# apchenstu/mvsnerf

Hardware: AMD Instinct MI355X
Metric: rendered rays/sec (1024-ray batch, 128 samples) (higher is better)
Workload: dtype f32; 1 GPU; config 2: 3 source views 512x640, 128 depth planes, pad 24 (volume 128x176x208x8), 1024 rays x 128 samples per step, MLP arithmetic fp32, render-only (volume pre-built); weights=mvsnerf-v0 checkpoint, volume=mvsnet-encode, parallelism=ray-sharded x1, no data-path collective

## Files before the change

mvsnerf_amd/csrc/mlp.hip:

```cpp
#include "common.h"
#include "mlp_layout.h"
#include "lds_dma.h"
#include "mlp_fp32_dev.h"
#include "knobs.h"
#include "sample_dev.h"
#include "composite_wave.h"
#include "march.h"

using namespace mlp;
typedef float f32x2 __attribute__((ext_vector_type(2)));

struct PackArgs {
    const float* w[11];
    const float* b[11];
    int F;
    float add;
};

__device__ inline void pack_segment(float* __restrict__ dst, const float* __restrict__ W, int ld, int col_off,
                                    int kmap, int steps, int nb, int F, int tid, int nthreads)
{
    const int total = steps * nb * 64;
    for (int i = tid; i < total; i += nthreads) {
        const int j = i & 3;
        const int lane = (i >> 2) & 63;
        const int rest = i >> 8;
        const int b = rest % nb, t = (rest / nb) * 4 + j;
        const int col = kmap_col(kmap, t, lane >> 5, F);
        const int row = b * 32 + (lane & 31);
        dst[i] = col < 0 ? 0.0f : W[(size_t)row * ld + col_off + col];
    }
}

template <bool FOLD>
__global__ __launch_bounds__(256) void mlp_pack_kernel(PackArgs a, float* __restrict__ packed)
{
    const Layout L = layout(a.F);
    const int tid = blockIdx.x * blockDim.x + threadIdx.x, nt = gridDim.x * blockDim.x;
    pack_segment(packed + L.biasw, a.w[6], a.F, 0, K_FEAT, L.fsteps, 4, a.F, tid, nt);
    pack_segment(packed + L.l0, a.w[0], PE_DIM, 0, K_PE, PE_STEPS, 4, a.F, tid, nt);
    pack_segment(packed + L.l1, a.w[1], WIDTH, 0, K_ACT, ACT_STEPS, 4, a.F, tid, nt);
    pack_segment(packed + L.l2, a.w[2], WIDTH, 0, K_ACT, ACT_STEPS, 4, a.F, tid, nt);
    pack_segment(packed + L.l3, a.w[3], WIDTH, 0, K_ACT, ACT_STEPS, 4, a.F, tid, nt);
    pack_segment(packed + L.l4, a.w[4], WIDTH, 0, K_ACT, ACT_STEPS, 4, a.F, tid, nt);
    pack_segment(packed + L.l5a, a.w[5], WIDTH + PE_DIM, 0, K_PE, PE_STEPS, 4, a.F, tid, nt);
    pack_segment(packed + L.l5b, a.w[5], WIDTH + PE_DIM, PE_DIM, K_ACT, ACT_STEPS, 4, a.F, tid, nt);
    pack_segment(packed + L.feat, a.w[7], WIDTH, 0, K_ACT, ACT_STEPS, 4, a.F, tid, nt);
    pack_segment(packed + L.views, a.w[9], WIDTH + 3, 0, K_VIEWS, VIEW_STEPS, 2, a.F, tid, nt);
    float* v = packed + L.vec;
    for (int i = tid; i < V_TOTAL; i += nt) {
        float x = 0.0f;
        if (i < V_VIEWS) {
            const int which = i >> 7, h = (i >> 6) & 1, q = i & 63;
            const float* src = which == 0 ? a.b[6] : which <= 6 ? a.b[which - 1] : a.b[7];
            x = src[act_n(q, h)];
        } else if (i < V_WA) {
            const int k = i - V_VIEWS;
            x = a.b[9][act_n(k & 31, k >> 5)];
        } else if (i < V_BA) {
            const int k = i - V_WA;
            x = a.w[8][act_n(k & 63, k >> 6)];
        } else if (i < V_WR) {
            x = (i == V_BA) ? a.b[8][0] : (FOLD && i == V_FOLD) ? 1.0f : (i == V_ADD) ? a.add : 0.0f;
        } else if (i < V_BR) {
            const int k = i - V_WR, c = k >> 6, h = (k >> 5) & 1, q = k & 31;
            x = a.w[10][c * 64 + act_n(q, h)];
        } else {
            const int c = i - V_BR;
            x = c < 3 ? a.b[10][c] : 0.0f;
        }
        v[i] = x;
    }
    if constexpr (FOLD) {
        const float* Wv = a.w[9];
        const float* Wf = a.w[7];
        float* fw = packed + fold_views_off(a.F);
        float* fb = packed + fold_bias_off(a.F);
        constexpr int total = (int)seg_floats(VIEW_STEPS, 2);
        for (int i = tid; i < total + 64; i += nt) {
            if (i < total) {
                const int lane = (i >> 2) & 63, rest = i >> 8;
                const int t = (rest >> 1) * 4 + (i & 3);
                const int col = kmap_col(K_VIEWS, t, lane >> 5, a.F);
                const float* wrow = Wv + (size_t)((rest & 1) * 32 + (lane & 31)) * (WIDTH + 3);
                float x = 0.0f;
                if (col >= WIDTH) {
                    x = wrow[col];
                } else if (col >= 0) {
                    double acc = 0.0;
                    for (int j = 0; j < WIDTH; ++j) acc = acc + (double)wrow[j] * (double)Wf[j * WIDTH + col];
                    x = (float)acc;
                }
                fw[i] = x;
            } else {
                const int k = i - total, n = act_n(k & 31, k >> 5);
                double acc = (double)a.b[9][n];
                for (int j = 0; j < WIDTH; ++j) acc = acc + (double)Wv[(size_t)n * (WIDTH + 3) + j] * (double)a.b[7][j];
                fb[k] = (float)acc;
            }
        }
    }
}

static size_t off16(int F) { return (layout(F).total + 3) & ~(size_t)3; }

extern "C" size_t mvsnerf_mlp_packed_floats(int F)
{
    if (F < 2 || F > MAX_F || (F & 1)) return 0;
    return off16(F);
}

extern "C" size_t mvsnerf_mlp_packed_fold_floats(int F)
{
    if (F < 2 || F > MAX_F || (F & 1)) return 0;
    return fold_total(F);
}

template <bool FOLD>
static int mlp_pack_impl(const float* const w[11], const float* const b[11], int F, float* packed, void* stream, float add = 0.0f)
{
    if (!w || !b || !packed) return MVSNERF_EINVAL;
    if (F < 2 || F > MAX_F || (F & 1)) return MVSNERF_EUNSUPPORTED;
    if (!mvs_aligned16(packed)) return MVSNERF_EALIGN;
    PackArgs a;
    for (int i = 0; i < 11; ++i) {
        if (!w[i] || !b[i]) return MVSNERF_EINVAL;
        a.w[i] = w[i]; a.b[i] = b[i];
    }
    a.F = F;
    a.add = add;
    mlp_pack_kernel<FOLD><<<64, 256, 0, (hipStream_t)stream>>>(a, packed);
    MVS_LAUNCH_CHECK();
    return MVSNERF_OK;
}

extern "C" int mvsnerf_mlp_pack(const float* const w[11], const float* const b[11], int F, float* packed, void* stream)
{
    return mlp_pack_impl<false>(w, b, F, packed, stream);
}

extern "C" int mvsnerf_mlp_pack_fold(const float* const w[11], const float* const b[11], int F, float* packed, void* stream)
{
    return mlp_pack_impl<true>(w, b, F, packed, stream);
}

extern "C" int mvsnerf_mlp_pack_fold_variant(const float* const w[11], const float* const b[11], int F, int variant, float* packed, void* stream)
{
    if (variant != 0 && variant != 1) return MVSNERF_EINVAL;
    return mlp_pack_impl<true>(w, b, F, packed, stream, variant ? 1.0f : 0.0f);
}

constexpr int WBUF_FLOATS = 16384;
constexpr int LDS_FLOATS = WBUF_FLOATS + V_TOTAL;

__device__ __forceinline__ void stage_weights(float* __restrict__ wbuf, const float* __restrict__ src, int n_floats, int tid)
{
    const f32x4* s = reinterpret_cast<const f32x4*>(src);
    f32x4* d = reinterpret_cast<f32x4*>(wbuf);
    const int n4 = n_floats >> 2;
#pragma unroll 4
    for (int i = tid; i < n4; i += 256) d[i] = s[i];
}

constexpr int SLAB_FLOATS = 8704;
constexpr int PIPE_LDS_FLOATS = 2 * SLAB_FLOATS + V_TOTAL;

struct RaymarchTileArgs {
    const float* vol; int D, H, W;
    const float* img; int V, IH, IW;
    const float* w2c; const float* Kmat;
    const float* pts; const float* rays_dir;
    float* feat; float* dirs_out;
    const float* z; int64_t N; int rays_per_tile;
    CompositeOut o;
};

__device__ __forceinline__ void tile_lookups(const unsigned tile, const RaymarchTileArgs& a, const float* __restrict__ ndc, int64_t P, int F,
                                             float* __restrict__ stage)
{
#pragma clang fp contract(off)
    const int tid = threadIdx.x, q = tid & 3;
    int r[2];
    bool live[2];
    unsigned p[2];
    ZfastTaps zt[2];
    ColorTap ct[2][2];
    f32x3 tap[2][2][4];
    f32x3 nn[2], pp[2];
#pragma unroll
    for (int ps = 0; ps < 2; ++ps) {
        r[ps] = ps * 64 + (tid >> 2);
        const int64_t p_raw = (int64_t)tile * 128 + r[ps];
        live[ps] = p_raw < P;
        p[ps] = (unsigned)(live[ps] ? p_raw : P - 1);
        nn[ps] = f32x3{ndc[p[ps] * 3 + 0], ndc[p[ps] * 3 + 1], ndc[p[ps] * 3 + 2]};
        pp[ps] = *reinterpret_cast<const f32x3*>(a.pts + p[ps] * 3);
    }
    const bool two = a.V > 4;
    const int vk[2] = {q < a.V ? q : a.V - 1, q + 4 < a.V ? q + 4 : a.V - 1};
    float Mv[2][12], Kv[2][9];
#pragma unroll
    for (int k = 0; k < 2; ++k)
        if (k == 0 || two) {
#pragma unroll
            for (int i = 0; i < 12; ++i) Mv[k][i] = a.w2c[vk[k] * 16 + i];
#pragma unroll
            for (int i = 0; i < 9; ++i) Kv[k][i] = a.Kmat[vk[k] * 9 + i];
        }
#pragma unroll
    for (int ps = 0; ps < 2; ++ps) zt[ps] = zfast_taps<true>(a.vol, a.D, a.H, a.W, nn[ps][0], nn[ps][1], nn[ps][2], q);
#pragma unroll
    for (int ps = 0; ps < 2; ++ps)
#pragma unroll
        for (int k = 0; k < 2; ++k)
            if (k == 0 || two) {
                ct[ps][k] = color_project(pp[ps][0], pp[ps][1], pp[ps][2], Mv[k], Kv[k], a.IW, a.IH);
                color_taps_nhwc4<true, f32x3>(a.img, vk[k], a.IH, a.IW, ct[ps][k], tap[ps][k]);
            }
#pragma unroll
    for (int ps = 0; ps < 2; ++ps) {
        float* srow = stage + r[ps] * F;
#pragma unroll
        for (int k = 0; k < 2; ++k)
            if ((k == 0 || two) && q + 4 * k < a.V) *reinterpret_cast<f32x4*>(srow + 8 + 16 * k + 4 * q) = color_row(ct[ps][k], tap[ps][k]);
        const f32x4 acc = zfast_fold_y0_lane(zt[ps]);
        if (q < 2) *reinterpret_cast<f32x4*>(srow + q * 4) = acc;
    }
}

__device__ __forceinline__ void tile_rows_out(const unsigned tile, float* __restrict__ feat, const float* __restrict__ stage, int64_t P, int F)
{
    const int64_t row0 = (int64_t)tile * 128;
    const int n4 = (int)(P - row0 < 128 ? P - row0 : 128) * (F / 4);
    f32x4* dst = reinterpret_cast<f32x4*>(feat + row0 * F);
    const f32x4* src = reinterpret_cast<const f32x4*>(stage);
    for (int i = threadIdx.x; i < n4; i += 256) dst[i] = src[i];
}

template <bool ALPHA_ONLY, bool SAVE, bool FUSED = false, int NR = 0>
__device__ __forceinline__ void mlp_fwd_pipe_tile(
    const unsigned tile, const float* __restrict__ packed, int F, const float* __restrict__ ndc, int ndc_stride,
    const float* __restrict__ feat, int feat_stride, const float* __restrict__ dirs, int dirs_stride,
    int64_t P, int S, float* __restrict__ raw, float* __restrict__ saved, long long* __restrict__ census, const RaymarchTileArgs* fa = nullptr)
{
    extern __shared__ __attribute__((aligned(16))) float lds[];
    long long t_start = 0, c_start = 0;
    if (census) { t_start = wall_clock64(); c_start = __builtin_amdgcn_s_memtime(); }
    int stamp_i = 4;
    auto stamp = [&]() { if (census && threadIdx.x == 0 && stamp_i < 16) census[tile * 16 + stamp_i] = wall_clock64(); ++stamp_i; };
    float* buf0 = lds;
    float* buf1 = lds + SLAB_FLOATS;
    float* vec = lds + 2 * SLAB_FLOATS;
    constexpr int G = 1;
    const Layout L = layout(F);
    const int tid = threadIdx.x, lane = tid & 63;
    const int wave = __builtin_amdgcn_readfirstlane(tid >> 6);
    const int half = lane >> 5;
    const int64_t p_raw = ((int64_t)tile * 4 + wave) * 32 + (lane & 31);
    const bool live = p_raw < P;
    const int64_t p = live ? p_raw : P - 1;
    float* sv = nullptr;
    if (SAVE) sv = saved + ((int64_t)tile * 4 + wave) * (SLOTS_SAVED * 64) + lane;
    auto save = [&](int slot, float v) { if (SAVE) sv[slot * 64] = v; };
    constexpr int HALF = (int)(ACT_STEPS / 2) * 4 * 64;

    constexpr int VEC_PER_THREAD = (V_TOTAL + 255) / 256;
    float vec_pre[VEC_PER_THREAD];
    if constexpr (FUSED) {
#pragma unroll
        for (int k = 0; k < VEC_PER_THREAD; ++k) vec_pre[k] = tid + 256 * k < V_TOTAL ? packed[L.vec + tid + 256 * k] : 0.0f;
    }
    slab_dma(buf0, packed + L.biasw, (int)seg_floats(L.fsteps, 4), wave, lane);
    const bool l0_first = !FUSED || seg_floats(L.fsteps, 4) + 128 * (size_t)F <= SLAB_FLOATS;
    float* stage = l0_first ? buf0 + seg_floats(L.fsteps, 4) : buf1;
    if (l0_first) slab_dma_c<(int)seg_floats(PE_STEPS, 4)>(buf1, packed + L.l0, wave, lane);
    if constexpr (FUSED) {
        tile_lookups(tile, *fa, ndc, P, F, stage);
#pragma unroll
        for (int k = 0; k < VEC_PER_THREAD; ++k)
            if (tid + 256 * k < V_TOTAL) vec[tid + 256 * k] = vec_pre[k];
    } else {
        for (int i = tid; i < V_TOTAL; i += 256) vec[i] = packed[L.vec + i];
    }
    const float px = ndc[p * ndc_stride + 0], py = ndc[p * ndc_stride + 1], pz = ndc[p * ndc_stride + 2];
    float fv[MAX_F / 2];
    if constexpr (FUSED) {
        slab_sync();
        const float* fp = stage + (wave * 32 + (lane & 31)) * F + half * (F / 2);
#pragma unroll
        for (int i = 0; i < MAX_F / 2; ++i) fv[i] = i < F / 2 ? fp[i] : 0.0f;
        tile_rows_out(tile, fa->feat, stage, P, F);
        if (!l0_first) {
            __syncthreads();
            slab_dma_c<(int)seg_floats(PE_STEPS, 4)>(buf1, packed + L.l0, wave, lane);
        }
    } else {
        const float* fp = feat + p * feat_stride + half * (F / 2);
#pragma unroll
        for (int i = 0; i < MAX_F / 2; ++i) fv[i] = i < F / 2 ? fp[i] : 0.0f;
    }
    float bias[64], h[64], pe_e[PE_STEPS];
    auto pe = [&](int g, int t) { return pe_e[t]; };
    auto hlo = [&](int g, int t) { return h[t]; };
    auto hhi = [&](int g, int t) { return h[32 + t]; };

    if constexpr (!FUSED) slab_sync();
    constexpr bool MAY_FOLD = !ALPHA_ONLY && !SAVE;
    bool fold = false;
    if constexpr (MAY_FOLD) {
        fold = __builtin_amdgcn_readfirstlane(__float_as_int(vec[V_FOLD])) != 0;
        if (fold && wave == 0) lds_dma_dword(packed + fold_bias_off(F), lds_byte_addr(vec + V_VIEWS), lane * 4);
    }
    const bool add = __builtin_amdgcn_readfirstlane(__float_as_int(vec[V_ADD])) != 0;
    stamp();
    {
        f32x16 acc[G][4];
        init_acc<4, G>(acc, vec + V_BIASG + half * 64);
        auto fb = [&](int g, int t) { return fv[t]; };
        switch (L.fsteps) {
            case 4:  gemm_stage<1, 4, G>(buf0, acc, lane, fb); break;
            case 8:  gemm_stage<2, 4, G>(buf0, acc, lane, fb); break;
            case 12: gemm_stage<3, 4, G>(buf0, acc, lane, fb); break;
            case 16: gemm_stage<4, 4, G>(buf0, acc, lane, fb); break;
            default: gemm_stage<5, 4, G>(buf0, acc, lane, fb); break;
        }
#pragma unroll
        for (int q = 0; q < 64; ++q) { bias[q] = acc[0][q >> 4][q & 15]; save(S_BM + q, bias[q]); }
        if (SAVE) {
#pragma unroll
            for (int t = 0; t < 16; ++t) save(S_FV + t, fv[t]);
            if (F > 32) {
#pragma unroll
                for (int t = 16; t < MAX_F / 2; ++t) save(S_FV_HI + t - 16, fv[t]);
            }
        }
    }
    stamp();
    {
        int half_o = half;
        asm("" : "+v"(half_o));
        pe_all(half_o, px, py, pz, pe_e);
    }
    if (SAVE) {
#pragma unroll
        for (int t = 0; t < PE_STEPS; ++t) save(S_E + t, pe_e[t]);
    }
    slab_sync();
    float* rdir_lds = buf0 + HALF + wave * 128;
    if constexpr (FUSED) {
        const unsigned ray_of_p = (unsigned)p / (unsigned)S;
        lds_dma_dword(fa->rays_dir, lds_byte_addr(rdir_lds), (ray_of_p * 3 + half) * 4);
        lds_dma_dword(fa->rays_dir, lds_byte_addr(rdir_lds + 64), (ray_of_p * 3 + 2) * 4);
    }
    {
        f32x16 acc[G][4];
        init_acc<4, G>(acc, vec + V_L0 + half * 64);
        gemm_stage<PE_STEPS / 4, 4, G>(buf1, acc, lane, pe, SlabUnder<HALF>{buf0, packed + L.l1, wave, lane});
        if (add) {
#pragma unroll
            for (int q = 0; q < 64; q += 2) {
                const f32x2 m2 = f32x2{acc[0][q >> 4][q & 15], acc[0][q >> 4][(q & 15) + 1]} + f32x2{bias[q], bias[q + 1]};
                h[q] = fmaxf(m2[0], 0.0f); h[q + 1] = fmaxf(m2[1], 0.0f);
            }
        } else {
#pragma unroll
            for (int q = 0; q < 64; q += 2) {
                const f32x2 m2 = f32x2{acc[0][q >> 4][q & 15], acc[0][q >> 4][(q & 15) + 1]} * f32x2{bias[q], bias[q + 1]};
                h[q] = fmaxf(m2[0], 0.0f); h[q + 1] = fmaxf(m2[1], 0.0f);
            }
        }
        if constexpr (SAVE) {
#pragma unroll
            for (int q = 0; q < 64; ++q) save(S_H + q, h[q]);
        }
    }
    stamp();
#pragma unroll 1
    for (int layer = 1; layer <= 4; ++layer) {
        const float* wl = packed + L.l1 + (size_t)(layer - 1) * seg_floats(ACT_STEPS, 4);
        f32x16 acc[G][4];
        slab_sync();
        init_acc<4, G>(acc, vec + V_L0 + 128 * layer + half * 64);
        gemm_stage<8, 4, G>(buf0, acc, lane, hlo, SlabUnder<HALF>{buf1, wl + HALF, wave, lane});
        slab_sync();
        gemm_stage<8, 4, G>(buf1, acc, lane, hhi, SlabUnder<HALF>{buf0, layer < 4 ? wl + 2 * HALF : packed + L.l5a, wave, lane});
        if (add) {
#pragma unroll
            for (int q = 0; q < 64; q += 2) {
                const f32x2 m2 = f32x2{acc[0][q >> 4][q & 15], acc[0][q >> 4][(q & 15) + 1]} + f32x2{bias[q], bias[q + 1]};
                h[q] = fmaxf(m2[0], 0.0f); h[q + 1] = fmaxf(m2[1], 0.0f);
            }
        } else {
#pragma unroll
            for (int q = 0; q < 64; q += 2) {
                const f32x2 m2 = f32x2{acc[0][q >> 4][q & 15], acc[0][q >> 4][(q & 15) + 1]} * f32x2{bias[q], bias[q + 1]};
                h[q] = fmaxf(m2[0], 0.0f); h[q + 1] = fmaxf(m2[1], 0.0f);
            }
        }
        if constexpr (SAVE) {
#pragma unroll
            for (int q = 0; q < 64; ++q) save(S_H + layer * 64 + q, h[q]);
        }
        stamp();
    }
    float sigma;
    {
        f32x16 acc[G][4];
        slab_sync();
        init_acc<4, G>(acc, vec + V_L0 + 128 * 5 + half * 64);
        gemm_stage<PE_STEPS / 4, 4, G>(buf0, acc, lane, pe, SlabUnder<HALF>{buf1, packed + L.l5b, wave, lane});
        slab_sync();
        gemm_stage<8, 4, G>(buf1, acc, lane, hlo, SlabUnder<HALF>{buf0, packed + L.l5b + HALF, wave, lane});
        slab_sync();
        if constexpr (SAVE) gemm_stage<8, 4, G>(buf0, acc, lane, hhi, SlabUnder<HALF>{buf1, packed + L.feat, wave, lane});
        else if constexpr (!ALPHA_ONLY) gemm_stage<8, 4, G>(buf0, acc, lane, hhi, SlabUnder<(int)seg_floats(VIEW_STEPS, 2)>{buf1, packed + (fold ? fold_views_off(F) : L.feat), wave, lane});
        else gemm_stage<8, 4, G>(buf0, acc, lane, hhi);
        if (add) {
#pragma unroll
            for (int q = 0; q < 64; q += 2) {
                const f32x2 m2 = f32x2{acc[0][q >> 4][q & 15], acc[0][q >> 4][(q & 15) + 1]} + f32x2{bias[q], bias[q + 1]};
                h[q] = fmaxf(m2[0], 0.0f); h[q + 1] = fmaxf(m2[1], 0.0f);
            }
        } else {
#pragma unroll
            for (int q = 0; q < 64; q += 2) {
                const f32x2 m2 = f32x2{acc[0][q >> 4][q & 15], acc[0][q >> 4][(q & 15) + 1]} * f32x2{bias[q], bias[q + 1]};
                h[q] = fmaxf(m2[0], 0.0f); h[q + 1] = fmaxf(m2[1], 0.0f);
            }
        }
        if constexpr (SAVE) {
#pragma unroll
            for (int q = 0; q < 64; ++q) save(S_H + 5 * 64 + q, h[q]);
        }
        const float* wa = vec + V_WA + half * 64;
        float part = 0.0f;
#pragma unroll
        for (int q = 0; q < 64; ++q) part = fmaf(wa[q], h[q], part);
        part += __shfl_xor(part, 32);
        sigma = part + vec[V_BA];
        if (!(ALPHA_ONLY && add)) sigma = fmaxf(sigma, 0.0f);
    }
    stamp();
    if (ALPHA_ONLY) {
        if (live && half == 0) raw[p_raw] = sigma;
        return;
    }
    if (!fold) {
        f32x16 acc[G][4];
        slab_sync();
        init_acc<4, G>(acc, vec + V_FEAT + half * 64);
        gemm_stage<8, 4, G>(buf1, acc, lane, hlo, SlabUnder<HALF>{buf0, packed + L.feat + HALF, wave, lane});
        slab_sync();
        gemm_stage<8, 4, G>(buf0, acc, lane, hhi, SlabUnder<(int)seg_floats(VIEW_STEPS, 2)>{buf1, packed + L.views, wave, lane});
#pragma unroll
        for (int q = 0; q < 64; ++q) { h[q] = acc[0][q >> 4][q & 15]; save(S_FE + q, h[q]); }
    }
    stamp();
    {
        int lane_o = lane;
        asm("" : "+v"(lane_o));
        const int64_t p_raw = ((int64_t)tile * 4 + wave) * 32 + (lane_o & 31);
        const bool live = p_raw < P;
        const int64_t p = live ? p_raw : P - 1;
        float z_pre = 0.0f;
        if constexpr (FUSED && NR > 0)
            if (tid < 128 && (int64_t)tile * 128 + tid < P) z_pre = fa->z[(int64_t)tile * 128 + tid];
        float d0, d1, d2;
        if constexpr (FUSED) {
            const int64_t ray = (unsigned)p / (unsigned)S;
            const float rdir[3] = {rdir_lds[lane & 31], rdir_lds[32 + (lane & 31)], rdir_lds[64 + (lane & 31)]};
            float rot[11];
#pragma unroll
            for (int i = 0; i < 11; ++i) rot[i] = fa->w2c[i];
            float d[3];
            dir_feature_of(rdir, rot, 1, d);
            d0 = d[0]; d1 = d[1]; d2 = d[2];
            if (live && half == 0 && p_raw == ray * S) { fa->dirs_out[ray * 3 + 0] = d0; fa->dirs_out[ray * 3 + 1] = d1; fa->dirs_out[ray * 3 + 2] = d2; }
        } else {
            const int64_t ray = p / S; d0 = dirs[ray * dirs_stride + 0]; d1 = dirs[ray * dirs_stride + 1]; d2 = dirs[ray * dirs_stride + 2];
        }
        f32x16 acc[G][2];
        slab_sync();
        init_acc<2, G>(acc, vec + V_VIEWS + half * 32);
        gemm_stage<VIEW_STEPS / 4, 2, G>(buf1, acc, lane, [&](int g, int t) {
            return t < ACT_STEPS ? h[t < ACT_STEPS ? t : 0] : t == ACT_STEPS ? (half ? d1 : d0) : t == ACT_STEPS + 1 ? (half ? 0.0f : d2) : 0.0f;
        });
        if (SAVE) {
#pragma unroll
            for (int q = 0; q < 32; ++q) save(S_HV + q, fmaxf(acc[0][q >> 4][q & 15], 0.0f));
            save(S_DR + 0, half ? d1 : d0);
            save(S_DR + 1, half ? 0.0f : d2);
        }
        float rgb[3];
#pragma unroll
        for (int c = 0; c < 3; ++c) {
            const float* wr = vec + V_WR + c * 64 + half * 32;
            float part = 0.0f;
#pragma unroll
            for (int q = 0; q < 32; ++q) part = fmaf(wr[q], fmaxf(acc[0][q >> 4][q & 15], 0.0f), part);
            part += __shfl_xor(part, 32);
            const float x = part + vec[V_BR + c];
            rgb[c] = 1.0f / (1.0f + expf(-x));
        }
        if (live && half == 0) *reinterpret_cast<f32x4*>(raw + p_raw * 4) = f32x4{rgb[0], rgb[1], rgb[2], sigma};
        if constexpr (FUSED && NR > 0) {
            if (half == 0) reinterpret_cast<f32x4*>(buf0)[wave * 32 + (lane_o & 31)] = f32x4{rgb[0], rgb[1], rgb[2], sigma};
            float* zs = buf0 + 4 * 128;
            if (tid < 128) zs[tid] = z_pre;
            __syncthreads();
            const f32x4* rs = reinterpret_cast<const f32x4*>(buf0);
            for (int rl = wave; rl < fa->rays_per_tile; rl += 4) {
                const int64_t ray = (int64_t)tile * fa->rays_per_tile + rl;
                if (ray >= fa->N) break;
                f32x4 rv[NR];
#pragma unroll
                for (int i = 0; i < NR; ++i) {
                    const int s = lane * NR + i;
                    rv[i] = s < S ? rs[rl * S + s] : f32x4{0, 0, 0, 0};
                }
                composite_wave<NR>(rv, zs + rl * S, ray, S, lane, fa->o);
            }
        }
    }
    if (census && tid == 0) {
        census[tile * 16 + 0] = t_start;
        census[tile * 16 + 1] = wall_clock64();
        census[tile * 16 + 2] = __builtin_amdgcn_s_getreg((4) | (0 << 6) | (31 << 11));
        census[tile * 16 + 3] = __builtin_amdgcn_s_getreg((20) | (0 << 6) | (31 << 11));
        census[tile * 16 + 13] = __builtin_amdgcn_s_memtime() - c_start;
    }
}

template <bool ALPHA_ONLY, bool SAVE>
__global__ __launch_bounds__(256, 2) void mlp_fwd_pipe_kernel(
    const float* __restrict__ packed, int F, const float* __restrict__ ndc, int ndc_stride,
    const float* __restrict__ feat, int feat_stride, const float* __restrict__ dirs, int dirs_stride,
    int64_t P, int S, float* __restrict__ raw, float* __restrict__ saved, long long* __restrict__ census)
{
    mlp_fwd_pipe_tile<ALPHA_ONLY, SAVE>(blockIdx.x, packed, F, ndc, ndc_stride, feat, feat_stride, dirs, dirs_stride, P, S, raw, saved, census);
}

template <bool ALPHA_ONLY>
__global__ __launch_bounds__(256, 2) void mlp_fwd_pipe_if_kernel(
    const float* __restrict__ packed, int F, const float* __restrict__ ndc, int ndc_stride,
    const float* __restrict__ feat, int feat_stride, const float* __restrict__ dirs, int dirs_stride,
    int64_t P, int S, float* __restrict__ raw, const int* __restrict__ run_if)
{
    if (*run_if == 0) return;
    const unsigned n_tiles = (unsigned)((P + 127) / 128);
    for (unsigned tile = blockIdx.x; tile < n_tiles; tile += gridDim.x) {
        mlp_fwd_pipe_tile<ALPHA_ONLY, false>(tile, packed, F, ndc, ndc_stride, feat, feat_stride, dirs, dirs_stride, P, S, raw, nullptr, nullptr);
        __syncthreads();
    }
}

template <bool ALPHA_ONLY>
__global__ __launch_bounds__(256, 2) void mlp_fwd_pipe_counted_kernel(
    const float* __restrict__ packed, int F, const float* __restrict__ ndc, const float* __restrict__ feat, const float* __restrict__ dirs,
    int cap, const int* __restrict__ count, float* __restrict__ raw, const int* __restrict__ run_if)
{
    if (run_if && *run_if == 0) return;
    const int n = mvs_counted_rows(count, cap);
    const unsigned n_tiles = ((unsigned)n + 127u) / 128u;
    for (unsigned tile = blockIdx.x; tile < n_tiles; tile += gridDim.x) {
        mlp_fwd_pipe_tile<ALPHA_ONLY, false>(tile, packed, F, ndc, 3, feat, F, dirs, 3, n, 1, raw, nullptr, nullptr);
        __syncthreads();
    }
}

template <bool AO>
static int launch_mlp_pipe_counted(const float* packed, int F, const float* ndc, const float* feat, const float* dirs, int cap, const int* count,
                                   float* raw, const int* run_if, hipStream_t st)
{
    const size_t lds_bytes = PIPE_LDS_FLOATS * sizeof(float);
    static unsigned long long cap_set = 0;
    if (int rc_ = mvs_raise_lds_cap(reinterpret_cast<const void*>(mlp_fwd_pipe_counted_kernel<AO>), (int)lds_bytes, &cap_set)) return rc_;
    const unsigned n_tiles = mvs_cdiv(cap, 128);
    mlp_fwd_pipe_counted_kernel<AO><<<n_tiles < 512u ? n_tiles : 512u, 256, lds_bytes, st>>>(packed, F, ndc, feat, dirs, cap, count, raw, run_if);
    MVS_LAUNCH_CHECK();
    return MVSNERF_OK;
}

int mvs_mlp_fwd_counted(const float* packed, int F, const float* ndc, const float* feat, const float* dirs, int64_t cap, const int* count,
                        int alpha_only, float* raw, const int* run_if, void* stream)
{
    if (!packed || !ndc || !feat || !raw || (!alpha_only && !dirs)) return MVSNERF_EINVAL;
    if (int rc = mvs_counted_args(count, cap)) return rc;
    if (F < 2 || F > MAX_F || (F & 1)) return MVSNERF_EUNSUPPORTED;
    if (!mvs_aligned16(packed) || !mvs_aligned16(raw)) return MVSNERF_EALIGN;
    if (cap == 0) return MVSNERF_OK;
    if (alpha_only) return launch_mlp_pipe_counted<true>(packed, F, ndc, feat, dirs, (int)cap, count, raw, run_if, (hipStream_t)stream);
    return launch_mlp_pipe_counted<false>(packed, F, ndc, feat, dirs, (int)cap, count, raw, run_if, (hipStream_t)stream);
}

extern "C" int mvsnerf_mlp_fwd_counted(const float* packed, int F, const float* ndc, const float* feat, const float* dirs, int64_t cap,
                                       const int* count, int alpha_only, float* raw, void* stream)
{
    return mvs_mlp_fwd_counted(packed, F, ndc, feat, dirs, cap, count, alpha_only, raw, nullptr, stream);
}

template <bool AO, bool SAVE>
static int launch_mlp_pipe(const float* packed, int F, const float* ndc, int ndc_stride, const float* feat, int feat_stride,
                           const float* dirs, int dirs_stride, int64_t P, int S, float* raw, hipStream_t st, float* saved = nullptr, long long* census = nullptr,
                           const int* run_if = nullptr)
{
    const size_t lds_bytes = PIPE_LDS_FLOATS * sizeof(float);
    if (run_if) {
        if constexpr (!SAVE) {
            static unsigned long long cap_if = 0;
            if (int rc_ = mvs_raise_lds_cap(reinterpret_cast<const void*>(mlp_fwd_pipe_if_kernel<AO>), (int)lds_bytes, &cap_if)) return rc_;
            const unsigned n_tiles = mvs_cdiv(P, 128);
            mlp_fwd_pipe_if_kernel<AO><<<n_tiles < 512u ? n_tiles : 512u, 256, lds_bytes, st>>>(packed, F, ndc, ndc_stride, feat, feat_stride, dirs, dirs_stride, P, S, raw, run_if);
            MVS_LAUNCH_CHECK();
            return MVSNERF_OK;
        } else {
            return MVSNERF_EINVAL;
        }
    }
    static unsigned long long lds_cap_set = 0;
    if (int rc_ = mvs_raise_lds_cap(reinterpret_cast<const void*>(mlp_fwd_pipe_kernel<AO, SAVE>), (int)lds_bytes, &lds_cap_set)) return rc_;
    mlp_fwd_pipe_kernel<AO, SAVE><<<mvs_cdiv(P, 128), 256, lds_bytes, st>>>(packed, F, ndc, ndc_stride, feat, feat_stride, dirs, dirs_stride, P, S, raw, saved, census);
    MVS_LAUNCH_CHECK();
    return MVSNERF_OK;
}

template <int NR>
__global__ __launch_bounds__(256, 2) void raymarch_fused_kernel(const float* __restrict__ packed, int F, const float* __restrict__ ndc, int64_t P, int S,
                                                                float* __restrict__ raw, RaymarchTileArgs fa)
{
    mlp_fwd_pipe_tile<false, false, true, NR>(blockIdx.x, packed, F, ndc, 3, nullptr, F, nullptr, 3, P, S, raw, nullptr, nullptr, &fa);
}

bool mvs_raymarch_fused_applies(const MarchBatch& b)
{
    if (b.packed_bf16 || b.packed_split || b.guard) return false;
    const int F = 8 + 4 * b.V;
    if (b.vol_layout != MVSNERF_VOL_HWDC || !b.vol || !b.imgs_nhwc4 || !b.w2c || !b.K || !b.packed || !b.pts || !b.ndc || !b.z || !b.rays_dir ||
        !b.feat || !b.dirs || !b.raw) return false;
    if (b.D < 1 || b.H < 1 || b.W < 1 || b.V < 1 || F > MAX_F || b.IH < 2 || b.IW < 2 || b.N < 1 || b.S < 1) return false;
    if (!mvs_aligned16(b.feat) || !mvs_aligned16(b.vol) || !mvs_aligned16(b.imgs_nhwc4) || !mvs_aligned16(b.packed) || !mvs_aligned16(b.raw)) return false;
    return gather_fits_32bit(b.D, b.H, b.W, b.V, b.IH, b.IW, b.N * b.S, F);
}

int mvs_raymarch_fused_fwd(const MarchBatch& b, hipStream_t st)
{
    const int F = 8 + 4 * b.V, S = b.S;
    const int64_t P = b.N * S;
    const RaymarchTileArgs fa{b.vol, b.D, b.H, b.W, b.imgs_nhwc4, b.V, b.IH, b.IW, b.w2c, b.K, b.pts, b.rays_dir, b.feat, b.dirs, b.z, b.N,
                              128 % S == 0 ? 128 / S : 0, CompositeOut{b.rgb_map, b.disp, b.acc, b.weights, b.depth, b.alpha, b.white_bkgd, nullptr}};
    const size_t lds_bytes = PIPE_LDS_FLOATS * sizeof(float);
    const unsigned grid = mvs_cdiv(P, 128);
    static unsigned long long cap[3] = {0, 0, 0};
#define MVS_FUSED(NR_)                                                                                                                 \
    do {                                                                                                                               \
        if (int rc_ = mvs_raise_lds_cap(reinterpret_cast<const void*>(raymarch_fused_kernel<NR_>), (int)lds_bytes, &cap[NR_])) return rc_; \
        raymarch_fused_kernel<NR_><<<grid, 256, lds_bytes, st>>>(b.packed, F, b.ndc, P, S, b.raw, fa);                               \
    } while (0)
    if (fa.rays_per_tile == 0) MVS_FUSED(0);
    else if (S <= 64) MVS_FUSED(1);
    else MVS_FUSED(2);
#undef MVS_FUSED
    MVS_LAUNCH_CHECK();
    if (fa.rays_per_tile == 0)
        return mvs_composite_fwd(b.raw, b.z, b.N, S, b.white_bkgd, b.rgb_map, b.disp, b.acc, b.weights, b.depth, b.alpha, nullptr, st);
    return MVSNERF_OK;
}

static int mlp_fwd_checked(const float* packed, int F, const float* ndc, int ndc_stride, const float* feat, int feat_stride,
                           const float* dirs, int dirs_stride, int64_t N, int S, int alpha_only, float* raw, void* stream, long long* census,
                           const int* run_if = nullptr)
{
    if (!packed || !ndc || !feat || !raw || N < 0 || S < 1 || feat_stride < F || ndc_stride < 3) return MVSNERF_EINVAL;
    if (!alpha_only && dirs_stride < 3) return MVSNERF_EINVAL;
    if (!alpha_only && !dirs) return MVSNERF_EINVAL;
    if (F < 2 || F > MAX_F || (F & 1)) return MVSNERF_EUNSUPPORTED;
    if (!mvs_aligned16(packed) || !mvs_aligned16(raw)) return MVSNERF_EALIGN;
    const int64_t P = N * S;
    if (P == 0) return MVSNERF_OK;
    hipStream_t st = (hipStream_t)stream;
    if (alpha_only) return launch_mlp_pipe<true, false>(packed, F, ndc, ndc_stride, feat, feat_stride, dirs, dirs_stride, P, S, raw, st, nullptr, census, run_if);
    return launch_mlp_pipe<false, false>(packed, F, ndc, ndc_stride, feat, feat_stride, dirs, dirs_stride, P, S, raw, st, nullptr, census, run_if);
}

int mvs_mlp_fwd_if(const float* packed, int F, const float* ndc, int ndc_stride, const float* feat, int feat_stride,
                   const float* dirs, int dirs_stride, int64_t N, int S, int alpha_only, float* raw, const int* run_if, void* stream)
{
    return mlp_fwd_checked(packed, F, ndc, ndc_stride, feat, feat_stride, dirs, dirs_stride, N, S, alpha_only, raw, stream, nullptr, run_if);
}

extern "C" int mvsnerf_mlp_fwd(const float* packed, int F, const float* ndc, int ndc_stride, const float* feat, int feat_stride,
                               const float* dirs, int dirs_stride, int64_t N, int S, int alpha_only, float* raw, void* stream)
{
    return mlp_fwd_checked(packed, F, ndc, ndc_stride, feat, feat_stride, dirs, dirs_stride, N, S, alpha_only, raw, stream, nullptr);
}

extern "C" int mvsnerf_mlp_fwd_census(const float* packed, int F, const float* ndc, int ndc_stride, const float* feat, int feat_stride,
                                      const float* dirs, int dirs_stride, int64_t N, int S, int alpha_only, float* raw, long long* census, void* stream)
{
    if (!census) return MVSNERF_EINVAL;
    return mlp_fwd_checked(packed, F, ndc, ndc_stride, feat, feat_stride, dirs, dirs_stride, N, S, alpha_only, raw, stream, census);
}

extern "C" int mvsnerf_mlp_fwd_train(const float* packed, int F, const float* ndc, int ndc_stride, const float* feat, int feat_stride,
                                     const float* dirs, int dirs_stride, int64_t N, int S, float* raw, float* saved, void* stream)
{
    if (!packed || !ndc || !feat || !dirs || !raw || !saved || N < 0 || S < 1 || feat_stride < F || ndc_stride < 3 || dirs_stride < 3) return MVSNERF_EINVAL;
    if (F < 2 || F > MAX_F || (F & 1)) return MVSNERF_EUNSUPPORTED;
    if (!mvs_aligned16(packed) || !mvs_aligned16(raw) || !mvs_aligned16(saved)) return MVSNERF_EALIGN;
    const int64_t P = N * S;
    if (P == 0) return MVSNERF_OK;
    return launch_mlp_pipe<false, true>(packed, F, ndc, ndc_stride, feat, feat_stride, dirs, dirs_stride, P, S, raw, (hipStream_t)stream, saved);
}

template <int VARIANT>
__global__ __launch_bounds__(64) void pe_operands_kernel(const float* __restrict__ ndc, float* __restrict__ out)
{
    const int lane = threadIdx.x, half = lane >> 5;
    const int64_t p = (int64_t)blockIdx.x * 32 + (lane & 31);
    const float px = ndc[p * 3 + 0], py = ndc[p * 3 + 1], pz = ndc[p * 3 + 2];
    float e[PE_STEPS];
    if constexpr (VARIANT == 0) {
#pragma unroll
        for (int t = 0; t < PE_STEPS; ++t) e[t] = pe_operand(t, half, px, py, pz);
    } else {
        pe_all(half, px, py, pz, e);
    }
#pragma unroll
    for (int t = 0; t < PE_STEPS; ++t) out[(p * PE_STEPS + t) * 2 + half] = e[t];
}

extern "C" int mvsnerf_pe_operands_fwd(const float* ndc, int64_t P, int variant, float* out, void* stream)
{
    if (!ndc || !out || P < 0 || (P & 31) || P / 32 > 0x7fffffff || (variant != 0 && variant != 1)) return MVSNERF_EINVAL;
    if (P == 0) return MVSNERF_OK;
    if (variant == 0) pe_operands_kernel<0><<<(unsigned)(P / 32), 64, 0, (hipStream_t)stream>>>(ndc, out);
    else pe_operands_kernel<1><<<(unsigned)(P / 32), 64, 0, (hipStream_t)stream>>>(ndc, out);
    MVS_LAUNCH_CHECK();
    return MVSNERF_OK;
}
```

mvsnerf_amd/csrc/mlp_fp32_dev.h:

```cpp
#pragma once
#include "common.h"
#include "lds_dma.h"

struct NoHook {
    static constexpr int STEPS = 0;
    __device__ __forceinline__ void operator()(int) const {}
};

template <int STEPS4, int NBLK, int G, typename BFN, typename HOOK = NoHook>
__device__ __forceinline__ void gemm_stage(const float* __restrict__ w, f32x16 (&acc)[G][NBLK], int lane, BFN bfn, HOOK under = HOOK())
{
    static_assert(HOOK::STEPS <= 3 * STEPS4, "the hook's pieces must fit under the GEMM's k-steps");
#pragma unroll
    for (int t4 = 0; t4 < STEPS4; ++t4) {
        f32x4 a[NBLK];
#pragma unroll
        for (int b = 0; b < NBLK; ++b)
            a[b] = *reinterpret_cast<const f32x4*>(w + ((t4 * NBLK + b) * 64 + lane) * 4);
#pragma unroll
        for (int j = 0; j < 4; ++j) {
            float bv[G];
#pragma unroll
            for (int g = 0; g < G; ++g) bv[g] = bfn(g, t4 * 4 + j);
#pragma unroll
            for (int b = 0; b < NBLK; ++b)
#pragma unroll
                for (int g = 0; g < G; ++g)
                    acc[g][b] = __builtin_amdgcn_mfma_f32_32x32x2f32(a[b][j], bv[g], acc[g][b], 0, 0, 0);
            if (j < 3 && t4 * 3 + j < HOOK::STEPS) {
                __builtin_amdgcn_sched_barrier(0);
                under(t4 * 3 + j);
                __builtin_amdgcn_sched_barrier(0);
            }
        }
    }
}

template <int NBLK, int G>
__device__ __forceinline__ void init_acc(f32x16 (&acc)[G][NBLK], const float* __restrict__ vec_h)
{
#pragma unroll
    for (int b = 0; b < NBLK; ++b)
#pragma unroll
        for (int r4 = 0; r4 < 4; ++r4) {
            const f32x4 v = *reinterpret_cast<const f32x4*>(vec_h + b * 16 + r4 * 4);
#pragma unroll
            for (int g = 0; g < G; ++g) {
                acc[g][b][r4 * 4 + 0] = v[0]; acc[g][b][r4 * 4 + 1] = v[1]; acc[g][b][r4 * 4 + 2] = v[2]; acc[g][b][r4 * 4 + 3] = v[3];
            }
        }
}

__device__ __forceinline__ float pe_sin_or_cos(float x, int want_cos)
{
    x = fminf(fmaxf(x, -65536.0f), 65536.0f);
    const float k = rintf(x * 0.63661977236758134f);
    float r = fmaf(k, -1.5703125f, x);
    r = fmaf(k, -4.837512969970703125e-4f, r);
    r = fmaf(k, -7.54978995489188e-8f, r);
    const float r2 = r * r;
    const float sp = fmaf(fmaf(-1.9515295891e-4f, r2, 8.3321608736e-3f), r2, -1.6666654611e-1f);
    const float sn = fmaf(sp * r2, r, r);
    const float cp = fmaf(fmaf(2.443315711809948e-5f, r2, -1.388731625493765e-3f), r2, 4.166664568298827e-2f);
    const float cs = fmaf(cp * r2, r2, fmaf(-0.5f, r2, 1.0f));
    const int q = (int)k + want_cos;
    const float v = (q & 1) ? cs : sn;
    return (q & 2) ? -v : v;
}

__device__ __forceinline__ float pe_operand(int t, int half, float px, float py, float pz)
{
    if (t == 0) return half ? py : px;
    if (t == 1) return half ? 0.0f : pz;
    const int j = t - 2, f = j / 3, c = j - 3 * f;
    const float x = (c == 0 ? px : c == 1 ? py : pz) * (float)(1 << f);
    return pe_sin_or_cos(x, half);
}

typedef float pe_f32x2 __attribute__((ext_vector_type(2)));
__device__ __forceinline__ void pe_sincos2(pe_f32x2 x, pe_f32x2& s, pe_f32x2& c)
{
    x[0] = fminf(fmaxf(x[0], -65536.0f), 65536.0f);
    x[1] = fminf(fmaxf(x[1], -65536.0f), 65536.0f);
    const pe_f32x2 kx = x * pe_f32x2{0.63661977236758134f, 0.63661977236758134f};
    const pe_f32x2 k = {rintf(kx[0]), rintf(kx[1])};
    auto fma2 = [](pe_f32x2 a, pe_f32x2 b, pe_f32x2 d) { return __builtin_elementwise_fma(a, b, d); };
    auto all = [](float v) { return pe_f32x2{v, v}; };
    pe_f32x2 r = fma2(k, all(-1.5703125f), x);
    r = fma2(k, all(-4.837512969970703125e-4f), r);
    r = fma2(k, all(-7.54978995489188e-8f), r);
    const pe_f32x2 r2 = r * r;
    const pe_f32x2 sp = fma2(fma2(all(-1.9515295891e-4f), r2, all(8.3321608736e-3f)), r2, all(-1.6666654611e-1f));
    const pe_f32x2 sn = fma2(sp * r2, r, r);
    const pe_f32x2 cp = fma2(fma2(all(2.443315711809948e-5f), r2, all(-1.388731625493765e-3f)), r2, all(4.166664568298827e-2f));
    const pe_f32x2 cs = fma2(cp * r2, r2, fma2(all(-0.5f), r2, all(1.0f)));
#pragma unroll
    for (int i = 0; i < 2; ++i) {
        const unsigned q = (unsigned)(int)k[i];
        const bool odd = q & 1u;
        s[i] = __uint_as_float(__float_as_uint(odd ? cs[i] : sn[i]) ^ ((q & 2u) << 30));
        c[i] = __uint_as_float(__float_as_uint(odd ? sn[i] : cs[i]) ^ (((q + 1u) & 2u) << 30));
    }
}

__device__ __forceinline__ void pe_all(int half, float px, float py, float pz, float (&e)[32])
{
    e[0] = half ? py : px;
    e[1] = half ? 0.0f : pz;
    const float co[3] = {px, py, pz};
    float x[16], sv[16], cv[16];
#pragma unroll
    for (int m = 0; m < 5; ++m) {
        const float scale = half ? (float)(2 << (2 * m)) : (float)(1 << (2 * m));
#pragma unroll
        for (int c = 0; c < 3; ++c) x[3 * m + c] = co[c] * scale;
    }
    x[15] = x[14];
#pragma unroll
    for (int i = 0; i < 16; i += 2) {
        pe_f32x2 s2, c2;
        pe_sincos2(pe_f32x2{x[i], x[i + 1]}, s2, c2);
        sv[i] = s2[0]; sv[i + 1] = s2[1]; cv[i] = c2[0]; cv[i + 1] = c2[1];
    }
#pragma unroll
    for (int m = 0; m < 5; ++m)
#pragma unroll
        for (int c = 0; c < 3; ++c) {
            const auto sw = __builtin_amdgcn_permlane32_swap(__float_as_uint(sv[3 * m + c]), __float_as_uint(cv[3 * m + c]), false, false);
            e[2 + 6 * m + c] = __uint_as_float(sw[0]);
            e[5 + 6 * m + c] = __uint_as_float(sw[1]);
        }
}

__device__ __forceinline__ void slab_dma(float* __restrict__ dst, const float* __restrict__ src, int n_floats, int wave, int lane)
{
    lds_dma<4>(dst, src, n_floats >> 8, wave, lane);
}
template <int N_FLOATS>
__device__ __forceinline__ void slab_dma_c(float* __restrict__ dst, const float* __restrict__ src, int wave, int lane)
{
    lds_dma_c<4, N_FLOATS / 256>(dst, src, wave, lane);
}

template <int N_FLOATS>
struct SlabUnder {
    static constexpr int STEPS = lds_dma_steps(4, N_FLOATS / 256);
    float* dst; const float* src; int wave, lane;
    __device__ __forceinline__ void operator()(int k) const { lds_dma_piece<4, N_FLOATS / 256>(dst, src, wave, lane, k); }
};

__device__ __forceinline__ void slab_sync()
{
    asm volatile("s_waitcnt vmcnt(0)" ::: "memory");
    __syncthreads();
}
```

Before: 4.797 million rays/s.

## Replace double-buffered weight slabs with a three-slot LDS ring in the MLP

Swaps the two large ping-pong LDS weight slabs for a three-slot ring of quarter-size chunks. Each 16-k-step GEMM quarter prefetches the chunk two ahead while computing, and the full __syncthreads is replaced by a barrier placed inside the GEMM schedule. A PIN mode keeps the LDS read address in a VGPR and advances it during the last k-steps. The view layer is split across two slots with an explicit MFMA bridge step. The aim is to hide weight-streaming latency and barrier stalls, at the cost of more frequent barriers and more complex slot indexing.

```diff
diff --git a/mvsnerf_amd/csrc/mlp.hip b/mvsnerf_amd/csrc/mlp.hip
--- a/mvsnerf_amd/csrc/mlp.hip
+++ b/mvsnerf_amd/csrc/mlp.hip
@@ -162,8 +162,9 @@
     for (int i = tid; i < n4; i += 256) d[i] = s[i];
 }
 
-constexpr int SLAB_FLOATS = 8704;
-constexpr int PIPE_LDS_FLOATS = 2 * SLAB_FLOATS + V_TOTAL;
+constexpr int RING_SLOT = 4352;
+constexpr int RING_Q = 4096;
+constexpr int PIPE_LDS_FLOATS = 4 * RING_SLOT + V_TOTAL;
 
 struct RaymarchTileArgs {
     const float* vol; int D, H, W;
@@ -237,7 +238,7 @@
     for (int i = threadIdx.x; i < n4; i += 256) dst[i] = src[i];
 }
 
-template <bool ALPHA_ONLY, bool SAVE, bool FUSED = false, int NR = 0>
+template <bool ALPHA_ONLY, bool SAVE, bool FUSED = false, int NR = 0, bool WALK = false>
 __device__ __forceinline__ void mlp_fwd_pipe_tile(
     const unsigned tile, const float* __restrict__ packed, int F, const float* __restrict__ ndc, int ndc_stride,
     const float* __restrict__ feat, int feat_stride, const float* __restrict__ dirs, int dirs_stride,
@@ -248,10 +249,14 @@
     if (census) { t_start = wall_clock64(); c_start = __builtin_amdgcn_s_memtime(); }
     int stamp_i = 4;
     auto stamp = [&]() { if (census && threadIdx.x == 0 && stamp_i < 16) census[tile * 16 + stamp_i] = wall_clock64(); ++stamp_i; };
-    float* buf0 = lds;
-    float* buf1 = lds + SLAB_FLOATS;
-    float* vec = lds + 2 * SLAB_FLOATS;
+    float* const slot0 = lds;
+    float* const slot1 = lds + RING_SLOT;
+    float* const slot2 = lds + 2 * RING_SLOT;
+    float* const xtra = lds + 3 * RING_SLOT;
+    float* vec = lds + 4 * RING_SLOT;
+    auto slot = [&](int c) { return lds + (c % 3) * RING_SLOT; };
     constexpr int G = 1;
+    constexpr bool PIN = !WALK;
     const Layout L = layout(F);
     const int tid = threadIdx.x, lane = tid & 63;
     const int wave = __builtin_amdgcn_readfirstlane(tid >> 6);
@@ -262,7 +267,7 @@
     float* sv = nullptr;
     if (SAVE) sv = saved + ((int64_t)tile * 4 + wave) * (SLOTS_SAVED * 64) + lane;
     auto save = [&](int slot, float v) { if (SAVE) sv[slot * 64] = v; };
-    constexpr int HALF = (int)(ACT_STEPS / 2) * 4 * 64;
+    const float* const wsrc = packed + L.l0;
 
     constexpr int VEC_PER_THREAD = (V_TOTAL + 255) / 256;
     float vec_pre[VEC_PER_THREAD];
@@ -270,10 +275,13 @@
 #pragma unroll
         for (int k = 0; k < VEC_PER_THREAD; ++k) vec_pre[k] = tid + 256 * k < V_TOTAL ? packed[L.vec + tid + 256 * k] : 0.0f;
     }
-    slab_dma(buf0, packed + L.biasw, (int)seg_floats(L.fsteps, 4), wave, lane);
-    const bool l0_first = !FUSED || seg_floats(L.fsteps, 4) + 128 * (size_t)F <= SLAB_FLOATS;
-    float* stage = l0_first ? buf0 + seg_floats(L.fsteps, 4) : buf1;
-    if (l0_first) slab_dma_c<(int)seg_floats(PE_STEPS, 4)>(buf1, packed + L.l0, wave, lane);
+    slab_dma(slot2, packed + L.biasw, (int)seg_floats(L.fsteps, 4), wave, lane);
+    const bool l0_first = !FUSED || seg_floats(L.fsteps, 4) + 128 * (size_t)F <= 2 * RING_SLOT;
+    float* stage = l0_first ? slot2 + seg_floats(L.fsteps, 4) : slot0;
+    if (l0_first) {
+        slab_dma_c<RING_Q>(slot0, wsrc, wave, lane);
+        slab_dma_c<RING_Q>(slot1, wsrc + RING_Q, wave, lane);
+    }
     if constexpr (FUSED) {
         tile_lookups(tile, *fa, ndc, P, F, stage);
 #pragma unroll
@@ -292,7 +300,8 @@
         tile_rows_out(tile, fa->feat, stage, P, F);
         if (!l0_first) {
             __syncthreads();
-            slab_dma_c<(int)seg_floats(PE_STEPS, 4)>(buf1, packed + L.l0, wave, lane);
+            slab_dma_c<RING_Q>(slot0, wsrc, wave, lane);
+            slab_dma_c<RING_Q>(slot1, wsrc + RING_Q, wave, lane);
         }
     } else {
         const float* fp = feat + p * feat_stride + half * (F / 2);
@@ -300,10 +309,6 @@
         for (int i = 0; i < MAX_F / 2; ++i) fv[i] = i < F / 2 ? fp[i] : 0.0f;
     }
     float bias[64], h[64], pe_e[PE_STEPS];
-    auto pe = [&](int g, int t) { return pe_e[t]; };
-    auto hlo = [&](int g, int t) { return h[t]; };
-    auto hhi = [&](int g, int t) { return h[32 + t]; };
-
     if constexpr (!FUSED) slab_sync();
     constexpr bool MAY_FOLD = !ALPHA_ONLY && !SAVE;
     bool fold = false;
@@ -318,11 +323,11 @@
         init_acc<4, G>(acc, vec + V_BIASG + half * 64);
         auto fb = [&](int g, int t) { return fv[t]; };
         switch (L.fsteps) {
-            case 4:  gemm_stage<1, 4, G>(buf0, acc, lane, fb); break;
-            case 8:  gemm_stage<2, 4, G>(buf0, acc, lane, fb); break;
-            case 12: gemm_stage<3, 4, G>(buf0, acc, lane, fb); break;
-            case 16: gemm_stage<4, 4, G>(buf0, acc, lane, fb); break;
-            default: gemm_stage<5, 4, G>(buf0, acc, lane, fb); break;
+            case 4:  gemm_stage<1, 4, G>(slot2, acc, lane, fb); break;
+            case 8:  gemm_stage<2, 4, G>(slot2, acc, lane, fb); break;
+            case 12: gemm_stage<3, 4, G>(slot2, acc, lane, fb); break;
+            case 16: gemm_stage<4, 4, G>(slot2, acc, lane, fb); break;
+            default: gemm_stage<5, 4, G>(slot2, acc, lane, fb); break;
         }
 #pragma unroll
         for (int q = 0; q < 64; ++q) { bias[q] = acc[0][q >> 4][q & 15]; save(S_BM + q, bias[q]); }
@@ -346,16 +351,20 @@
         for (int t = 0; t < PE_STEPS; ++t) save(S_E + t, pe_e[t]);
     }
     slab_sync();
-    float* rdir_lds = buf0 + HALF + wave * 128;
+    float* rdir_lds = xtra + wave * 128;
     if constexpr (FUSED) {
         const unsigned ray_of_p = (unsigned)p / (unsigned)S;
         lds_dma_dword(fa->rays_dir, lds_byte_addr(rdir_lds), (ray_of_p * 3 + half) * 4);
         lds_dma_dword(fa->rays_dir, lds_byte_addr(rdir_lds + 64), (ray_of_p * 3 + 2) * 4);
     }
+    auto pe_q = [&](int q) { return [&pe_e, q](int g, int t) { return pe_e[16 * q + t]; }; };
+    auto h_q = [&](int q) { return [&h, q](int g, int t) { return h[16 * q + t]; }; };
+    RingAddr wad{lds_byte_addr(slot(0)) + lane * 16, slot(0)};
     {
         f32x16 acc[G][4];
         init_acc<4, G>(acc, vec + V_L0 + half * 64);
-        gemm_stage<PE_STEPS / 4, 4, G>(buf1, acc, lane, pe, SlabUnder<HALF>{buf0, packed + L.l1, wave, lane});
+        gemm_ring<4, 4, G, true, PIN>(wad, slot(1), acc, lane, pe_q(0), RingUnder<RING_Q, false>{slot(2), wsrc + 2 * RING_Q, wave, lane});
+        gemm_ring<4, 4, G, true, PIN>(wad, slot(2), acc, lane, pe_q(1), RingUnder<RING_Q>{slot(3), wsrc + 3 * RING_Q, wave, lane});
         if (add) {
 #pragma unroll
             for (int q = 0; q < 64; q += 2) {
@@ -376,14 +385,17 @@
     }
     stamp();
 #pragma unroll 1
-    for (int layer = 1; layer <= 4; ++layer) {
-        const float* wl = packed + L.l1 + (size_t)(layer - 1) * seg_floats(ACT_STEPS, 4);
+    for (int layer = 1, ph = 2; layer <= 4; ++layer, ph = ph == 2 ? 0 : ph + 1) {
+        const float* wl = wsrc + (size_t)(4 * layer - 2) * RING_Q;
+        if constexpr (!PIN) wad.w = lds + ph * RING_SLOT;
         f32x16 acc[G][4];
-        slab_sync();
         init_acc<4, G>(acc, vec + V_L0 + 128 * layer + half * 64);
-        gemm_stage<8, 4, G>(buf0, acc, lane, hlo, SlabUnder<HALF>{buf1, wl + HALF, wave, lane});
-        slab_sync();
-        gemm_stage<8, 4, G>(buf1, acc, lane, hhi, SlabUnder<HALF>{buf0, layer < 4 ? wl + 2 * HALF : packed + L.l5a, wave, lane});
+#pragma unroll
+        for (int q = 0; q < 4; ++q) {
+            auto mod3 = [](int s) { return s >= 6 ? s - 6 : s >= 3 ? s - 3 : s; };
+            gemm_ring<4, 4, G, true, PIN>(wad, lds + mod3(ph + q + 1) * RING_SLOT, acc, lane, h_q(q),
+                                           RingUnder<RING_Q>{lds + mod3(ph + q + 2) * RING_SLOT, wl + (q + 2) * RING_Q, wave, lane});
+        }
         if (add) {
 #pragma unroll
             for (int q = 0; q < 64; q += 2) {
@@ -406,15 +418,22 @@
     float sigma;
     {
         f32x16 acc[G][4];
-        slab_sync();
         init_acc<4, G>(acc, vec + V_L0 + 128 * 5 + half * 64);
-        gemm_stage<PE_STEPS / 4, 4, G>(buf0, acc, lane, pe, SlabUnder<HALF>{buf1, packed + L.l5b, wave, lane});
-        slab_sync();
-        gemm_stage<8, 4, G>(buf1, acc, lane, hlo, SlabUnder<HALF>{buf0, packed + L.l5b + HALF, wave, lane});
-        slab_sync();
-        if constexpr (SAVE) gemm_stage<8, 4, G>(buf0, acc, lane, hhi, SlabUnder<HALF>{buf1, packed + L.feat, wave, lane});
-        else if constexpr (!ALPHA_ONLY) gemm_stage<8, 4, G>(buf0, acc, lane, hhi, SlabUnder<(int)seg_floats(VIEW_STEPS, 2)>{buf1, packed + (fold ? fold_views_off(F) : L.feat), wave, lane});
-        else gemm_stage<8, 4, G>(buf0, acc, lane, hhi);
+        gemm_ring<4, 4, G, true, PIN>(wad, slot(19), acc, lane, pe_q(0), RingUnder<RING_Q>{slot(20), wsrc + 20 * RING_Q, wave, lane});
+        gemm_ring<4, 4, G, true, PIN>(wad, slot(20), acc, lane, pe_q(1), RingUnder<RING_Q>{slot(21), wsrc + 21 * RING_Q, wave, lane});
+        gemm_ring<4, 4, G, true, PIN>(wad, slot(21), acc, lane, h_q(0), RingUnder<RING_Q>{slot(22), wsrc + 22 * RING_Q, wave, lane});
+        gemm_ring<4, 4, G, true, PIN>(wad, slot(22), acc, lane, h_q(1), RingUnder<RING_Q>{slot(23), wsrc + 23 * RING_Q, wave, lane});
+        if constexpr (SAVE) {
+            gemm_ring<4, 4, G, true, PIN>(wad, slot(23), acc, lane, h_q(2), RingUnder<RING_Q>{slot(24), wsrc + 24 * RING_Q, wave, lane});
+            gemm_ring<4, 4, G, false, PIN>(wad, nullptr, acc, lane, h_q(3), RingUnder<RING_Q>{slot(25), wsrc + 25 * RING_Q, wave, lane});
+        } else if constexpr (!ALPHA_ONLY) {
+            const float* w24 = fold ? packed + fold_views_off(F) : wsrc + 24 * RING_Q;
+            gemm_ring<4, 4, G, true, PIN>(wad, slot(23), acc, lane, h_q(2), RingUnder<RING_SLOT>{slot(24), w24, wave, lane});
+            gemm_ring<4, 4, G, false, PIN>(wad, nullptr, acc, lane, h_q(3), RingUnder<RING_SLOT>{slot(25), w24 + (fold ? RING_SLOT : RING_Q), wave, lane});
+        } else {
+            gemm_ring<4, 4, G, true, PIN>(wad, slot(23), acc, lane, h_q(2), RingUnder<0>{nullptr, nullptr, wave, lane});
+            gemm_ring<4, 4, G, false, PIN>(wad, nullptr, acc, lane, h_q(3));
+        }
         if (add) {
 #pragma unroll
             for (int q = 0; q < 64; q += 2) {
@@ -447,11 +466,12 @@
     }
     if (!fold) {
         f32x16 acc[G][4];
-        slab_sync();
         init_acc<4, G>(acc, vec + V_FEAT + half * 64);
-        gemm_stage<8, 4, G>(buf1, acc, lane, hlo, SlabUnder<HALF>{buf0, packed + L.feat + HALF, wave, lane});
-        slab_sync();
-        gemm_stage<8, 4, G>(buf0, acc, lane, hhi, SlabUnder<(int)seg_floats(VIEW_STEPS, 2)>{buf1, packed + L.views, wave, lane});
+        wad = RingAddr{lds_byte_addr(slot(24)) + lane * 16, slot(24)};
+        gemm_ring<4, 4, G, true, PIN>(wad, slot(25), acc, lane, h_q(0), RingUnder<RING_Q>{slot(26), wsrc + 26 * RING_Q, wave, lane});
+        gemm_ring<4, 4, G, true, PIN>(wad, slot(26), acc, lane, h_q(1), RingUnder<RING_Q>{slot(27), wsrc + 27 * RING_Q, wave, lane});
+        gemm_ring<4, 4, G, true, PIN>(wad, slot(27), acc, lane, h_q(2), RingUnder<RING_SLOT>{slot(28), packed + L.views, wave, lane});
+        gemm_ring<4, 4, G, false, PIN>(wad, nullptr, acc, lane, h_q(3), RingUnder<RING_SLOT>{slot(29), packed + L.views + RING_SLOT, wave, lane});
 #pragma unroll
         for (int q = 0; q < 64; ++q) { h[q] = acc[0][q >> 4][q & 15]; save(S_FE + q, h[q]); }
     }
@@ -480,11 +500,19 @@
             const int64_t ray = p / S; d0 = dirs[ray * dirs_stride + 0]; d1 = dirs[ray * dirs_stride + 1]; d2 = dirs[ray * dirs_stride + 2];
         }
         f32x16 acc[G][2];
-        slab_sync();
         init_acc<2, G>(acc, vec + V_VIEWS + half * 32);
-        gemm_stage<VIEW_STEPS / 4, 2, G>(buf1, acc, lane, [&](int g, int t) {
-            return t < ACT_STEPS ? h[t < ACT_STEPS ? t : 0] : t == ACT_STEPS ? (half ? d1 : d0) : t == ACT_STEPS + 1 ? (half ? 0.0f : d2) : 0.0f;
-        });
+        float* const va = MAY_FOLD && fold ? slot(24) : slot(28);
+        float* const vb = MAY_FOLD && fold ? slot(25) : slot(29);
+        auto vop = [&](int t) { return t < ACT_STEPS ? h[t < ACT_STEPS ? t : 0] : t == ACT_STEPS ? (half ? d1 : d0) : t == ACT_STEPS + 1 ? (half ? 0.0f : d2) : 0.0f; };
+        gemm_stage<8, 2, G>(va, acc, lane, [&](int g, int t) { return vop(t); }, RingUnder<0>{nullptr, nullptr, wave, lane});
+        {
+            const f32x4 a8[2] = {*reinterpret_cast<const f32x4*>(va + (16 * 64 + lane) * 4), *reinterpret_cast<const f32x4*>(vb + lane * 4)};
+#pragma unroll
+            for (int j = 0; j < 4; ++j)
+#pragma unroll
+                for (int b = 0; b < 2; ++b) acc[0][b] = __builtin_amdgcn_mfma_f32_32x32x2f32(a8[b][j], vop(32 + j), acc[0][b], 0, 0, 0);
+        }
+        gemm_stage<8, 2, G>(vb + 256, acc, lane, [&](int g, int t) { return vop(36 + t); });
         if (SAVE) {
 #pragma unroll
             for (int q = 0; q < 32; ++q) save(S_HV + q, fmaxf(acc[0][q >> 4][q & 15], 0.0f));
@@ -504,11 +532,11 @@
         }
         if (live && half == 0) *reinterpret_cast<f32x4*>(raw + p_raw * 4) = f32x4{rgb[0], rgb[1], rgb[2], sigma};
         if constexpr (FUSED && NR > 0) {
-            if (half == 0) reinterpret_cast<f32x4*>(buf0)[wave * 32 + (lane_o & 31)] = f32x4{rgb[0], rgb[1], rgb[2], sigma};
-            float* zs = buf0 + 4 * 128;
+            if (half == 0) reinterpret_cast<f32x4*>(xtra + 512)[wave * 32 + (lane_o & 31)] = f32x4{rgb[0], rgb[1], rgb[2], sigma};
+            float* zs = xtra + 512 + 4 * 128;
             if (tid < 128) zs[tid] = z_pre;
             __syncthreads();
-            const f32x4* rs = reinterpret_cast<const f32x4*>(buf0);
+            const f32x4* rs = reinterpret_cast<const f32x4*>(xtra + 512);
             for (int rl = wave; rl < fa->rays_per_tile; rl += 4) {
                 const int64_t ray = (int64_t)tile * fa->rays_per_tile + rl;
                 if (ray >= fa->N) break;
@@ -549,7 +577,7 @@
     if (*run_if == 0) return;
     const unsigned n_tiles = (unsigned)((P + 127) / 128);
     for (unsigned tile = blockIdx.x; tile < n_tiles; tile += gridDim.x) {
-        mlp_fwd_pipe_tile<ALPHA_ONLY, false>(tile, packed, F, ndc, ndc_stride, feat, feat_stride, dirs, dirs_stride, P, S, raw, nullptr, nullptr);
+        mlp_fwd_pipe_tile<ALPHA_ONLY, false, false, 0, true>(tile, packed, F, ndc, ndc_stride, feat, feat_stride, dirs, dirs_stride, P, S, raw, nullptr, nullptr);
         __syncthreads();
     }
 }
@@ -563,7 +591,7 @@
     const int n = mvs_counted_rows(count, cap);
     const unsigned n_tiles = ((unsigned)n + 127u) / 128u;
     for (unsigned tile = blockIdx.x; tile < n_tiles; tile += gridDim.x) {
-        mlp_fwd_pipe_tile<ALPHA_ONLY, false>(tile, packed, F, ndc, 3, feat, F, dirs, 3, n, 1, raw, nullptr, nullptr);
+        mlp_fwd_pipe_tile<ALPHA_ONLY, false, false, 0, true>(tile, packed, F, ndc, 3, feat, F, dirs, 3, n, 1, raw, nullptr, nullptr);
         __syncthreads();
     }
 }
diff --git a/mvsnerf_amd/csrc/mlp_fp32_dev.h b/mvsnerf_amd/csrc/mlp_fp32_dev.h
--- a/mvsnerf_amd/csrc/mlp_fp32_dev.h
+++ b/mvsnerf_amd/csrc/mlp_fp32_dev.h
@@ -30,6 +30,50 @@
             if (j < 3 && t4 * 3 + j < HOOK::STEPS) {
                 __builtin_amdgcn_sched_barrier(0);
                 under(t4 * 3 + j);
+                __builtin_amdgcn_sched_barrier(0);
+            }
+        }
+    }
+}
+
+typedef const __attribute__((address_space(3))) f32x4* lds_f32x4_ptr;
+struct RingAddr {
+    unsigned wa; const float* w;
+};
+template <int STEPS4, int NBLK, int G, bool NEXT, bool PIN, typename BFN, typename HOOK = NoHook>
+__device__ __forceinline__ void gemm_ring(RingAddr& ra, const float* w_next, f32x16 (&acc)[G][NBLK], int lane, BFN bfn, HOOK under = HOOK())
+{
+    static_assert(HOOK::STEPS <= 3 * STEPS4 - (NEXT && PIN ? 1 : 0), "the hook's pieces must fit under the GEMM's k-steps");
+    if constexpr (!PIN) {
+        gemm_stage<STEPS4, NBLK, G>(ra.w, acc, lane, bfn, under);
+        if (NEXT) ra.w = w_next;
+        return;
+    }
+#pragma unroll
+    for (int t4 = 0; t4 < STEPS4; ++t4) {
+        f32x4 a[NBLK];
+#pragma unroll
+        for (int b = 0; b < NBLK; ++b)
+            a[b] = *reinterpret_cast<lds_f32x4_ptr>(ra.wa + (t4 * NBLK + b) * 1024);
+#pragma unroll
+        for (int j = 0; j < 4; ++j) {
+            float bv[G];
+#pragma unroll
+            for (int g = 0; g < G; ++g) bv[g] = bfn(g, t4 * 4 + j);
+#pragma unroll
+            for (int b = 0; b < NBLK; ++b)
+#pragma unroll
+                for (int g = 0; g < G; ++g)
+                    acc[g][b] = __builtin_amdgcn_mfma_f32_32x32x2f32(a[b][j], bv[g], acc[g][b], 0, 0, 0);
+            if (j < 3 && t4 * 3 + j < HOOK::STEPS) {
+                __builtin_amdgcn_sched_barrier(0);
+                under(t4 * 3 + j);
+                __builtin_amdgcn_sched_barrier(0);
+            }
+            if (NEXT && PIN && t4 == STEPS4 - 1 && j == 2) {
+                __builtin_amdgcn_sched_barrier(0);
+                ra.wa = lds_byte_addr(w_next) + lane * 16;
+                asm volatile("" : "+v"(ra.wa));
                 __builtin_amdgcn_sched_barrier(0);
             }
         }
@@ -154,3 +198,21 @@
     asm volatile("s_waitcnt vmcnt(0)" ::: "memory");
     __syncthreads();
 }
+
+__device__ __forceinline__ void ring_barrier()
+{
+    asm volatile("s_waitcnt vmcnt(0)" ::: "memory");
+    __builtin_amdgcn_s_barrier();
+}
+
+template <int N_FLOATS, bool BAR = true>
+struct RingUnder {
+    static constexpr int PIECES = lds_dma_steps(4, N_FLOATS / 256);
+    static constexpr int STEPS = PIECES + (BAR ? 1 : 0);
+    float* dst; const float* src; int wave, lane;
+    __device__ __forceinline__ void operator()(int k) const
+    {
+        if (BAR && k == 0) { ring_barrier(); return; }
+        if constexpr (PIECES > 0) lds_dma_piece<4, N_FLOATS / 256>(dst, src, wave, lane, k - (BAR ? 1 : 0));
+    }
+};
```

Measured after the change: 4.791 million rays/s. Within noise of the previous version (-0.1%).
